# VinAIResearch/COMBAT

Hardware: AMD Instinct MI355X
Metric: images/sec per alternated generator+surrogate step, CIFAR-10 bs=128, 1/2/4/8 GPU (higher is better)
Workload: dtype bf16; 1 GPU; train_generator.py --dataset cifar10 --pc 0.5 --noise_rate 0.08: alternated PreActResNet18 surrogate + UNet generator step (Phase C + Phase G, both Nesterov-SGD updates), bs=128 per GPU, on-device augmentation on; per_gpu_batch=128, global_batch=128, parallelism=dp1 (RCCL all-reduce of netC grads in Phase C, netG grads in Phase G), losses_finite=True, deterministic=True

## Files before the change

### combat_amd/build.py

```python
import importlib.util
import os
import subprocess
import sys
from concurrent.futures import ThreadPoolExecutor

HERE = os.path.dirname(os.path.abspath(__file__))
ROOT = os.path.dirname(HERE)
CSRC = os.path.join(HERE, "csrc")
OBJ = os.path.join(CSRC, "_obj")
LIB = os.path.join(HERE, "libcombat_hip.so")
SOURCES = ["capi.cpp", "plan.cpp", "comm.cpp", "conv_gemm.hip", "conv3x3.hip", "conv3x3_dma.hip", "conv_gather_dma.hip", "conv_k8.hip", "conv_wgrad.hip", "conv_wgrad3x3.hip", "conv_wgrad3x3_dma.hip", "norm.hip", "elementwise.hip", "trigger.hip", "head.hip", "warp.hip"]
HIPCC = os.environ.get("HIPCC", "/opt/rocm/bin/hipcc")
FLAGS = ["--offload-arch=gfx950", "-O3", "-std=c++17", "-fPIC", "-munsafe-fp-atomics", "-Wno-unused-result", "-Wno-inline-asm",
         "-I" + os.path.join(ROOT, "include"), "-I" + CSRC] + os.environ.get("COMBAT_HIPCC_FLAGS", "").split()


def _newer(target, deps):
    if not os.path.exists(target):
        return True
    t = os.path.getmtime(target)
    return any(os.path.getmtime(d) > t for d in deps)


def check_counted_waits(lib=LIB, verbose=True):
    spec = importlib.util.spec_from_file_location("check_counted_waits", os.path.join(ROOT, "tools", "check_counted_waits.py"))
    mod = importlib.util.module_from_spec(spec)
    spec.loader.exec_module(mod)
    res = mod.check_file(lib)
    if verbose or not res.ok():
        print(res.report(), flush=True)
    if not res.ok():
        raise RuntimeError("counted-wait check failed: %d error(s), first: %s at 0x%x: %s"
                           % (len(res.errors), res.errors[0].kernel, res.errors[0].addr, res.errors[0].text))
    return res


def build(force=False, verbose=True):
    os.makedirs(OBJ, exist_ok=True)
    headers = [os.path.join(ROOT, "include", "combat_hip.h"), os.path.join(CSRC, "common.hpp"), os.path.join(CSRC, "conv_common.hpp"), os.path.join(CSRC, "conv_dma_epilogue.hpp"), os.path.join(CSRC, "plan.hpp")]
    jobs = []
    objs = []
    for src in SOURCES:
        s = os.path.join(CSRC, src)
        o = os.path.join(OBJ, os.path.splitext(src)[0] + ".o")
        objs.append(o)
        if force or _newer(o, [s] + headers):
            cmd = [HIPCC] + FLAGS + (["-x", "hip"] if src.endswith(".cpp") else []) + ["-c", s, "-o", o]
            jobs.append(cmd)

    def run(cmd):
        if verbose:
            print(" ".join(cmd), flush=True)
        subprocess.run(cmd, check=True)

    if jobs:
        with ThreadPoolExecutor(max_workers=min(4, len(jobs))) as ex:
            list(ex.map(run, jobs))
    if jobs or force or _newer(LIB, objs):
        tmp = LIB + ".unchecked"
        if os.path.exists(LIB):
            os.remove(LIB)
        run([HIPCC, "--offload-arch=gfx950", "-shared", "-fPIC", "-o", tmp] + objs)
        check_counted_waits(tmp, verbose)
        os.replace(tmp, LIB)
    return LIB


if __name__ == "__main__":
    print(build(force="--force" in sys.argv))
```

### combat_amd/csrc/conv_common.hpp

```cpp
#pragma once
#include "common.hpp"
#include <type_traits>

int conv3x3_pick(const combat_conv_args *a);
int conv3x3_stats_layout(const combat_conv_args *a, int tile, int *rows, int *rows_per_image);
int conv3x3_launch(const combat_conv_args *a, int tile, hipStream_t st);
int conv3x3d_pick(const combat_conv_args *a);
int conv3x3d_stats_layout(const combat_conv_args *a, int tile, int *rows, int *rows_per_image);
int conv3x3d_launch(const combat_conv_args *a, int tile, hipStream_t st);
int conv_gather_dma_bn(const combat_conv_args *a);
bool conv_gather_dma_parity_split(const combat_conv_args *a);
bool conv_c8_ok(const combat_conv_args *a);
int conv_c8_launch(const combat_conv_args *a, hipStream_t st);
bool conv_k8_ok(const combat_conv_args *a);
int conv_k8_launch(const combat_conv_args *a, hipStream_t st);
int conv_gather_dma_launch(const combat_conv_args *a, hipStream_t st);
int conv_gather_dma_pair_launch(const combat_conv_args *a, const combat_conv_args *b, hipStream_t st);
long conv_gather_dma_workspace(const combat_conv_args *a);
int conv_wgrad3x3_try(const combat_wgrad_args *a, hipStream_t st);
int conv_wgrad3x3_dma_try(const combat_wgrad_args *a, hipStream_t st);
long conv_wgrad3x3_dma_workspace(const combat_wgrad_args *a);
int conv_wgrad3x3_dma_reduce(const combat_wgrad_args *a, hipStream_t st);

template <int BM, int BN, int WGM_ = 0>
struct TileCfg {
    static constexpr int WGM = WGM_ ? WGM_ : ((BN == 16) ? 4 : 2);
    static constexpr int WGN = 4 / WGM;
    static constexpr int WM = BM / WGM;
    static constexpr int WN = BN / WGN;
    static constexpr int FM = WM / 16;
    static constexpr int FN = WN / 16;
    static constexpr int A_ITERS = BM / 32;
    static constexpr int B_ITERS = (BN + 31) / 32;
    static constexpr int EPS = BN + 4;
    static constexpr int STAGE_BYTES = 2 * (BM + BN) * 128;
    static constexpr int EP_BYTES = BM * EPS * 4;
    static constexpr int SMEM = STAGE_BYTES > EP_BYTES ? STAGE_BYTES : EP_BYTES;
    static constexpr int NC = BN / 8;
    static constexpr int RPT = BM * NC / 256;
    static constexpr int SG = BM / 4;
};

template <typename T, typename RowMap>
__device__ __forceinline__ void conv_epilogue(unsigned char *smem, const f32x4_t (&acc)[T::FN][T::FM],
                                              const combat_conv_args &a, int n0, int PQ, RowMap row_to_m,
                                              int part_row) {
    const int tid = threadIdx.x, lane = tid & 63, wid = tid >> 6;
    const int wave_m = wid % T::WGM, wave_n = wid / T::WGM;
    float *ep = reinterpret_cast<float *>(smem);
    {
        const int fr = lane & 15, fq = lane >> 4;
#pragma unroll
        for (int i = 0; i < T::FN; ++i)
#pragma unroll
            for (int j = 0; j < T::FM; ++j) {
                const int n = wave_n * T::WN + i * 16 + fq * 4;
                const int row = wave_m * T::WM + j * 16 + fr;
                *reinterpret_cast<f32x4_t *>(ep + row * T::EPS + n) = acc[i][j];
            }
    }
    __syncthreads();

    const int K = a.K;
    const int cc = tid % T::NC, rgrp = tid / T::NC;
    const int n = n0 + cc * 8;
    const bool n_ok = n < K;
    float bias8[8];
    if (a.bias && n_ok) load8f(a.bias + n, bias8);
    float s1[8], s2[8];
#pragma unroll
    for (int e = 0; e < 8; ++e) s1[e] = s2[e] = 0.f;
    __bf16 *__restrict__ dst = reinterpret_cast<__bf16 *>(a.dst);
    __bf16 *__restrict__ act_dst = reinterpret_cast<__bf16 *>(a.act_dst);
    float asc[8], ash[8];
    if (act_dst && n_ok) {
        load8f(a.act_scale + n, asc);
        load8f(a.act_shift + n, ash);
    }

    auto tail = [&](auto shared_tag) {
    constexpr bool tab_shared = decltype(shared_tag)::value;
    float msc[8], msh[8], hrs[8], hmn[8];
    if (a.mask_x && n_ok && tab_shared) {
        if (a.mask_scale) {
            load8f(a.mask_scale + n, msc);
            load8f(a.mask_shift + n, msh);
        }
        if ((a.stats_kind & 3) == 2) {
            load8f(a.xh_rstd + n, hrs);
            load8f(a.xh_mean + n, hmn);
        }
    }
    constexpr int RB = T::RPT < 4 ? T::RPT : 4;
#pragma unroll
    for (int pb = 0; pb < T::RPT; pb += RB) {
        int mrow[RB];
        uint4 l_pre[RB], l_x[RB], l_post[RB];
#pragma unroll
        for (int q = 0; q < RB; ++q) {
            const int row = rgrp * T::RPT + pb + q;
            const int m = n_ok ? row_to_m(row) : -1;
            mrow[q] = m;
            if (m >= 0) {
                const size_t off = (size_t)m * K + n;
                if (a.add_pre) l_pre[q] = *reinterpret_cast<const uint4 *>(reinterpret_cast<const __bf16 *>(a.add_pre) + off);
                if (a.mask_x) l_x[q] = *reinterpret_cast<const uint4 *>(reinterpret_cast<const __bf16 *>(a.mask_x) + off);
                if (a.add_post) l_post[q] = *reinterpret_cast<const uint4 *>(reinterpret_cast<const __bf16 *>(a.add_post) + off);
            }
        }
#pragma unroll
        for (int q = 0; q < RB; ++q) {
            const int m = mrow[q];
            if (m < 0) continue;
            const int row = rgrp * T::RPT + pb + q;
            float v[8];
            load8f(ep + row * T::EPS + cc * 8, v);
            const size_t off = (size_t)m * K + n;
            if (a.bias) {
#pragma unroll
                for (int e = 0; e < 8; ++e) v[e] += bias8[e];
            }
            if (a.add_pre) {
                float t[8];
                unpack8(l_pre[q], t);
#pragma unroll
                for (int e = 0; e < 8; ++e) v[e] += t[e];
            }
            float xm[8];
            if (a.mask_x) {
                unpack8(l_x[q], xm);
                if constexpr (!tab_shared) {
                    const int g = (m / PQ) * a.mask_group_stride;
                    if (a.mask_scale) {
                        load8f(a.mask_scale + g + n, msc);
                        load8f(a.mask_shift + g + n, msh);
                    }
                    if ((a.stats_kind & 3) == 2) {
                        load8f(a.xh_rstd + g + n, hrs);
                        load8f(a.xh_mean + g + n, hmn);
                    }
                }
                if (a.mask_scale) {
#pragma unroll
                    for (int e = 0; e < 8; ++e) {
                        const float qv = a.mask_activated ? xm[e] : fmaf(xm[e], msc[e], msh[e]);
                        float d = qv > 0.f ? 1.f : a.mask_slope;
                        if (a.mask_mul_scale) d *= msc[e];
                        v[e] *= d;
                    }
                } else {
#pragma unroll
                    for (int e = 0; e < 8; ++e) v[e] *= xm[e] > 0.f ? 1.f : a.mask_slope;
                }
            }
            if (a.add_post) {
                float t[8];
                unpack8(l_post[q], t);
#pragma unroll
                for (int e = 0; e < 8; ++e) v[e] += t[e];
            }
            if (a.tanh_out) {
#pragma unroll
                for (int e = 0; e < 8; ++e) v[e] = tanhf(v[e]);
            }
            const uint4 packed = pack8(v);
            if (dst) *reinterpret_cast<uint4 *>(dst + off) = packed;
            if (act_dst) {
                float t[8];
                unpack8(packed, t);
#pragma unroll
                for (int e = 0; e < 8; ++e) {
                    const float q = fmaf(t[e], asc[e], ash[e]);
                    t[e] = q > 0.f ? q : q * a.act_slope;
                }
                *reinterpret_cast<uint4 *>(act_dst + off) = pack8(t);
// ... 43 lines not shown
```

### combat_amd/csrc/conv_wgrad.hip

```cpp
#include "conv_common.hpp"
#include "plan.hpp"

namespace {

struct WgradParams {
    combat_wgrad_args a;
    int M, PQ, ntaps, tiles_k, tiles_c, split, pix_per_split;
    float *ws;
};

template <int BMC, int BNC>
struct WCfg {
    static constexpr int WGK = (BNC == 16) ? 4 : (BMC == 16 ? 1 : 2);
    static constexpr int WGC = 4 / WGK;
    static constexpr int WK = BMC / WGK;
    static constexpr int WC = BNC / WGC;
    static constexpr int FK = WK / 16;
    static constexpr int FC = WC / 16;
    static constexpr int SK = (BMC + 16) * 2;
    static constexpr int SC = (BNC + 16) * 2;
    static constexpr int CHK = BMC / 8;
    static constexpr int CHC = BNC / 8;
    static constexpr int ITK = (64 * CHK + 255) / 256;
    static constexpr int ITC = (64 * CHC + 255) / 256;
// ... 389 lines not shown
    p.ws = (p.split > 1 && p.a.workspace && p.a.workspace_bytes >= need) ? reinterpret_cast<float *>(p.a.workspace) : nullptr;
    if (combat_deterministic() && p.split > 1 && !p.ws) return COMBAT_EINVAL;
    COMBAT_LAUNCH(conv_wgrad_c8_kernel, dim3((unsigned)(p.tiles_k * p.split)), dim3(256), SMEM, st, p);
    CB_LAUNCH_CHECK();
    if (p.ws) {
        const int groups = p.split >= 32 ? 16 : 1;
        float *part = nullptr;
        if (combat_deterministic() && groups > 1) {
            const long extra = (long)groups * p.tiles_k * per_tile * 4;
            if (p.a.workspace_bytes >= need + extra) part = p.ws + need / 4;
        }
        const int g1 = combat_deterministic() && !part ? 1 : groups;
        COMBAT_LAUNCH(conv_wgrad_c8_reduce_kernel, dim3((per_tile + 255) / 256, p.tiles_k, g1), dim3(256), 0, st, (const float *)p.ws,
                           p.a.dw, p.tiles_k, p.split, per_tile, p.a.k_real, 9 * p.a.c_real, part);
        CB_LAUNCH_CHECK();
        if (part) {
            COMBAT_LAUNCH(conv_wgrad_c8_reduce_kernel, dim3((per_tile + 255) / 256, p.tiles_k, 1), dim3(256), 0, st, (const float *)part,
                               p.a.dw, p.tiles_k, groups, per_tile, p.a.k_real, 9 * p.a.c_real, (float *)nullptr);
            CB_LAUNCH_CHECK();
        }
    }
    return COMBAT_OK;
}

__global__ __launch_bounds__(256) void wgrad_slab_reduce_kernel(const float *__restrict__ ws, float *__restrict__ dw, int split,
                                                                int ntaps, int tiles_k, int tiles_c, int bmc, int bnc, int k_real,
                                                                int c_real, int C) {
    const long e = (long)blockIdx.x * 256 + threadIdx.x;
    if (e >= (long)k_real * ntaps * c_real) return;
    const int c = (int)(e % c_real), tap = (int)((e / c_real) % ntaps), n = (int)(e / ((long)c_real * ntaps));
    const int tile_k = n / bmc, row = n - tile_k * bmc;
    const size_t tile_elems = (size_t)bmc * bnc, sstride = (size_t)ntaps * tiles_k * tiles_c * tile_elems;
    float total = 0.f;
    for (int half = 0; half < 2; ++half) {
        const int cs = c + half * c_real;
        if (half && (c_real >= C || cs >= C || cs >= 2 * c_real)) break;
        const int tile_c = cs / bnc, col = cs - tile_c * bnc;
        const float *src = ws + (((size_t)tap * tiles_k + tile_k) * tiles_c + tile_c) * tile_elems + (size_t)row * bnc + col;
        float s0 = 0.f, s1 = 0.f, s2 = 0.f, s3 = 0.f;
        int sp = 0;
        for (; sp + 4 <= split; sp += 4) {
            s0 += src[(size_t)sp * sstride];
            s1 += src[(size_t)(sp + 1) * sstride];
            s2 += src[(size_t)(sp + 2) * sstride];
            s3 += src[(size_t)(sp + 3) * sstride];
        }
        for (; sp < split; ++sp) s0 += src[(size_t)sp * sstride];
        total += (s0 + s1) + (s2 + s3);
    }
    dw[e] += total;
}

template <int BMC, int BNC>
int64_t generic_slab_bytes(const combat_wgrad_args &a, int split) {
    const long tiles_k = (a.K + BMC - 1) / BMC, tiles_c = (a.C + BNC - 1) / BNC;
    return (int64_t)split * a.R * a.S * tiles_k * tiles_c * BMC * BNC * 4;
}

template <int BMC, int BNC>
int launch(WgradParams p, hipStream_t st) {
    using T = WCfg<BMC, BNC>;
    static bool attr_set = false;
    auto kern = conv_wgrad_kernel<BMC, BNC>;
    if (!attr_set) {
        if (hipFuncSetAttribute(reinterpret_cast<const void *>(kern), hipFuncAttributeMaxDynamicSharedMemorySize,
                                T::SMEM) != hipSuccess)
            return COMBAT_ELAUNCH;
        attr_set = true;
    }
    p.tiles_k = (p.a.K + BMC - 1) / BMC;
    p.tiles_c = (p.a.C + BNC - 1) / BNC;
    int split = p.a.split;
    const int ktiles = (p.M + 63) / 64;
    if (split <= 0) {
        const int base = p.tiles_k * p.tiles_c * p.ntaps;
        split = ((BMC == 16 ? 2304 : 256) + base - 1) / base;
        const int max_split = (ktiles + 3) / 4;
        if (split > max_split) split = max_split;
        if (split < 1) split = 1;
    }
    if (split > ktiles) split = ktiles;
    p.pix_per_split = ((ktiles + split - 1) / split) * 64;
    p.split = (p.M + p.pix_per_split - 1) / p.pix_per_split;
    const long blocks = (long)p.tiles_k * p.tiles_c * p.ntaps * p.split;
    p.ws = nullptr;
    if (combat_deterministic() && p.split > 1) {
        const int64_t need = generic_slab_bytes<BMC, BNC>(p.a, p.split);
        if (!p.a.workspace || p.a.workspace_bytes < need) return COMBAT_EINVAL;
        p.ws = reinterpret_cast<float *>(p.a.workspace);
    }
    COMBAT_LAUNCH(kern, dim3((unsigned)blocks), dim3(256), T::SMEM, st, p);
    CB_LAUNCH_CHECK();
    if (p.ws) {
        const long elems = (long)p.a.k_real * p.ntaps * p.a.c_real;
        COMBAT_LAUNCH(wgrad_slab_reduce_kernel, dim3((unsigned)((elems + 255) / 256)), dim3(256), 0, st, (const float *)p.ws, p.a.dw,
                      p.split, p.ntaps, p.tiles_k, p.tiles_c, BMC, BNC, p.a.k_real, p.a.c_real, p.a.C);
        CB_LAUNCH_CHECK();
    }
    return COMBAT_OK;
}

template <int BMC, int BNC>
int generic_split(const combat_wgrad_args &a) {
    const long M = (long)a.N * a.P * a.Q;
    const int ktiles = (int)((M + 63) / 64), ntaps = a.R * a.S;
    const int tiles_k = (a.K + BMC - 1) / BMC, tiles_c = (a.C + BNC - 1) / BNC;
    int split = a.split > 0 ? a.split : 0;
    if (split <= 0) {
        const int base = tiles_k * tiles_c * ntaps;
        split = ((BMC == 16 ? 2304 : 256) + base - 1) / base;
        const int max_split = (ktiles + 3) / 4;
        if (split > max_split) split = max_split;
        if (split < 1) split = 1;
    }
    if (split > ktiles) split = ktiles;
    const int pix_per_split = ((ktiles + split - 1) / split) * 64;
    return (int)((M + pix_per_split - 1) / pix_per_split);
}

bool c8_applies(const combat_wgrad_args *a) {
    return a->split >= 0 && a->C == 8 && a->R == 3 && (a->K & 63) == 0 && !a->pro_scale && !a->pro_act;
}

int64_t c8_workspace(const combat_wgrad_args &a) {
    const long M = (long)a.N * a.P * a.Q;
    const int ktiles = (int)((M + 63) / 64), tiles_k = a.K / 64;
    int split = a.split;
    if (split <= 0) {
        split = (256 + tiles_k - 1) / tiles_k;
        const int max_split = (ktiles + 3) / 4;
        if (split > max_split) split = max_split;
        if (split < 1) split = 1;
    }
    if (split > ktiles) split = ktiles;
    const int pix_per_split = ((ktiles + split - 1) / split) * 64;
    const long nsplit = (M + pix_per_split - 1) / pix_per_split;
    if (nsplit <= 1) return 0;
    const int64_t per_tile = 64 * 9 * a.c_real * 4;
    return tiles_k * nsplit * per_tile + (nsplit >= 32 ? 16 * tiles_k * per_tile : 0);
}

int64_t generic_workspace(const combat_wgrad_args &a) {
    if (a.C <= 16) return generic_slab_bytes<64, 16>(a, generic_split<64, 16>(a));
    if (a.K <= 16) return generic_slab_bytes<16, 64>(a, generic_split<16, 64>(a));
    if (a.C % 128 == 0 && a.K % 128 == 0) return generic_slab_bytes<128, 128>(a, generic_split<128, 128>(a));
    return generic_slab_bytes<64, 64>(a, generic_split<64, 64>(a));
}

}

extern "C" int64_t combat_conv_wgrad_workspace_bytes(const combat_wgrad_args *a) {
    if (!a) return 0;
    const int64_t dma = a->split >= 0 ? (int64_t)conv_wgrad3x3_dma_workspace(a) : 0;
    if (dma > 0 || !combat_deterministic()) return dma;
    return c8_applies(a) ? c8_workspace(*a) : generic_workspace(*a);
}

static int validate_wgrad_args(const combat_wgrad_args *a) {
    if (!a || !a->src || !a->dy || !a->dw) return COMBAT_EINVAL;
    if (a->N <= 0 || a->H <= 0 || a->W <= 0 || a->P <= 0 || a->Q <= 0) return COMBAT_EINVAL;
    if (a->C < 8 || (a->C & 7) || a->K < 8 || (a->K & 7)) return COMBAT_EINVAL;
    if (a->R != a->S || (a->R != 1 && a->R != 3)) return COMBAT_EINVAL;
    if (a->stride != 1 && a->stride != 2) return COMBAT_EINVAL;
    if (a->c_real <= 0 || a->c_real > a->C || a->k_real <= 0 || a->k_real > a->K) return COMBAT_EINVAL;
    if ((a->pro_scale == nullptr) != (a->pro_shift == nullptr)) return COMBAT_EINVAL;
    if ((long)a->N * a->P * a->Q > 0x7fffffffL / 8) return COMBAT_EINVAL;
    return COMBAT_OK;
}

extern "C" int combat_conv_wgrad_reduce(const combat_wgrad_args *a, void *stream) {
    COMBAT_PLAN_HOOK(combat_conv_wgrad_reduce, a);
    if (validate_wgrad_args(a) != COMBAT_OK) return COMBAT_EINVAL;
    if (a->split < 0 || !a->defer_reduce) return COMBAT_OK;
    return conv_wgrad3x3_dma_reduce(a, as_stream(stream));
}

extern "C" int combat_conv_wgrad(const combat_wgrad_args *a, void *stream) {
    COMBAT_PLAN_HOOK(combat_conv_wgrad, a);
    if (validate_wgrad_args(a) != COMBAT_OK) return COMBAT_EINVAL;
    WgradParams p;
    p.a = *a;
    p.ws = nullptr;
    p.PQ = a->P * a->Q;
    p.M = (int)((long)a->N * p.PQ);
    p.ntaps = a->R * a->S;
    hipStream_t st = as_stream(stream);
    if (a->split >= 0) {
        int rc = conv_wgrad3x3_dma_try(a, st);
        if (rc <= 0) return rc;
    }
    if (a->reduce_first) {
        const int rc = combat_conv_wgrad_reduce(a->reduce_first, stream);
        if (rc != COMBAT_OK) return rc;
    }
    if (a->split >= 0 && !combat_deterministic()) {
        const int rc = conv_wgrad3x3_try(a, st);
        if (rc <= 0) return rc;
    }
    if (a->split < 0) p.a.split = 0;
    if (c8_applies(a)) return launch_c8(p, st);
    if (a->C <= 16) return launch<64, 16>(p, st);
    if (a->K <= 16) return launch<16, 64>(p, st);
    if (a->C % 128 == 0 && a->K % 128 == 0) return launch<128, 128>(p, st);
    return launch<64, 64>(p, st);
}
```

### combat_amd/csrc/conv_wgrad3x3_dma.hip

```cpp
#include "conv_common.hpp"
#include <stdlib.h>

namespace {

typedef __attribute__((address_space(3))) void lds_void_t;
constexpr unsigned kOob = 0x40000000u;

struct W3dParams {
    combat_wgrad_args a;
    int TW, TH, TI, HWP, HH, HROWS, hpw, tw_shift, th_shift;
    int tiles_x, tiles_y, ntiles, tiles_k, tiles_c, split, per;
    unsigned x_bytes, dy_bytes;
    float *ws;
    const float *red_ws;
    float *red_dw;
    int red_base, red_tiles_c, red_split, red_k_real, red_c_real, red_pad;
    unsigned long long *stamps;
};

#ifdef COMBAT_STAMPS
static unsigned long long *g_stamps_wgrad_host = nullptr;
extern "C" int combat_debug_set_stamps_wgrad(void *p) { g_stamps_wgrad_host = (unsigned long long *)p; return 0; }
#define WCLK() __builtin_readcyclecounter()
#else
// ... 423 lines not shown
__global__ __launch_bounds__(512, 1) void conv_wgrad3x3_dma_kernel(const W3dParams p) { wgrad3x3_dma_body<HPW, NS, RED>(p); }

template <int HPW, int NS, bool RED>
int launch_w3d_red(const W3dParams &p, int blocks, hipStream_t st) {
    constexpr int stage = 8192 + HPW * 8192;
    constexpr int ep = 64 * 68 * 4;
    constexpr int smem = NS * stage > ep ? NS * stage : ep;
    auto kern = conv_wgrad3x3_dma_kernel<HPW, NS, RED>;
    static bool attr = false;
    if (!attr) {
        if (hipFuncSetAttribute(reinterpret_cast<const void *>(kern), hipFuncAttributeMaxDynamicSharedMemorySize, smem) != hipSuccess)
            return COMBAT_ELAUNCH;
        attr = true;
    }
    COMBAT_LAUNCH(kern, dim3(blocks), dim3(512), smem, st, p);
    CB_LAUNCH_CHECK();
    return COMBAT_OK;
}

template <int HPW, int NS>
int launch_w3d(const W3dParams &p, int blocks, hipStream_t st) {
    return p.red_ws ? launch_w3d_red<HPW, NS, true>(p, blocks, st) : launch_w3d_red<HPW, NS, false>(p, blocks, st);
}

bool w3d_geometry(const combat_wgrad_args *a, W3dParams &p, int &smem) {
    if (!(a->R == 3 && a->S == 3 && a->stride == 1 && a->pad == 1 && a->P == a->H && a->Q == a->W)) return false;
    if (a->pro_scale || a->pro_act) return false;
    if (a->C < 64 || (a->C & 63) || a->K < 64 || (a->K & 63) || a->c_real != a->C) return false;
    const int W = a->W, H = a->H;
    const int TW = W < 16 ? W : 16;
    const int TH = H < 64 / TW ? H : 64 / TW;
    const int TI = 64 / (TW * TH);
    if (TW < 2 || TI < 1 || TW * TH * TI != 64) return false;
    p.a = *a;
    p.TW = TW; p.TH = TH; p.TI = TI;
    p.HWP = TW + 2; p.HH = TH + 2; p.HROWS = TI * p.HH * p.HWP;
    p.hpw = (p.HROWS + 63) / 64;
    p.tw_shift = ilog2_exact(TW); p.th_shift = ilog2_exact(TH);
    if (p.tw_shift < 0 || p.th_shift < 0 || W % TW || H % TH) return false;
    const long xb = (long)a->N * H * W * a->C * 2, db = (long)a->N * H * W * a->K * 2;
    if (xb >= (long)kOob || db >= (long)kOob) return false;
    p.x_bytes = (unsigned)xb; p.dy_bytes = (unsigned)db;
    p.tiles_x = W / TW; p.tiles_y = H / TH;
    p.ntiles = p.tiles_x * p.tiles_y * ((a->N + TI - 1) / TI);
    p.tiles_k = a->K / 64; p.tiles_c = a->C / 64;
    smem = 0;
    return p.hpw >= 2 && p.hpw <= 4;
}

int pick_split(const combat_wgrad_args *a, const W3dParams &p, bool with_ws) {
    const int base = p.tiles_k * p.tiles_c;
    int split = a->split;
    if (split <= 0) {
        static const int ws_wgs = getenv("COMBAT_WGRAD_WGS") ? atoi(getenv("COMBAT_WGRAD_WGS")) : 128;
        const int by_cus = ((with_ws ? ws_wgs : 256) + base - 1) / base;
        const int by_atomics = 164 / base > 0 ? 164 / base : 1;
        split = with_ws || by_cus < by_atomics ? by_cus : by_atomics;
        const int by_work = (p.ntiles + 3) / 4;
        if (split > by_work) split = by_work;
        if (split < 1) split = 1;
    }
    if (split > p.ntiles) split = p.ntiles;
    const int per = (p.ntiles + split - 1) / split;
    return (p.ntiles + per - 1) / per;
}

}

long conv_wgrad3x3_dma_workspace(const combat_wgrad_args *a) {
    W3dParams p;
    int smem;
    if (!w3d_geometry(a, p, smem)) return 0;
    const int split = pick_split(a, p, true);
    return split > 1 ? (long)split * p.tiles_k * p.tiles_c * 9 * 4096 * 4 : 0;
}

namespace {
bool w3d_plan(const combat_wgrad_args *a, W3dParams &p) {
    int smem;
    if (!w3d_geometry(a, p, smem)) return false;
    const int base = p.tiles_k * p.tiles_c;
    int split = pick_split(a, p, true);
    const bool use_ws = split > 1 && a->workspace && a->workspace_bytes >= (long)split * base * 9 * 4096 * 4;
    if (!use_ws) split = pick_split(a, p, false);
    p.ws = use_ws ? reinterpret_cast<float *>(a->workspace) : nullptr;
    p.per = (p.ntiles + split - 1) / split;
    p.split = (p.ntiles + p.per - 1) / p.per;
    return true;
}

int launch_reduce(const combat_wgrad_args *a, const W3dParams &p, hipStream_t st) {
    const int base = p.tiles_k * p.tiles_c;
    static const bool env_det = getenv("COMBAT_WGRAD_DET_REDUCE") != nullptr;
    const bool det = combat_deterministic();
    const bool atomics = !env_det && (!det || base >= 4);
    if (atomics) {
        const long e4 = (long)base * 9 * 1024;
        int groups = (int)(512 / ((e4 + 255) / 256));
        if (groups < 1 || det) groups = 1;
        if (groups > p.split) groups = p.split;
        COMBAT_LAUNCH(wgrad3x3_reduce_kernel, dim3((unsigned)((e4 + 255) / 256), groups), dim3(256), 0, st, p.ws, a->dw, base,
                           p.tiles_c, p.split, a->k_real, a->c_real);
    } else {
        COMBAT_LAUNCH(wgrad3x3_reduce_det_kernel, dim3(256), dim3(256), 0, st, (const float *)p.ws, a->dw, base, p.tiles_c, p.split,
                           a->k_real, a->c_real);
    }
    CB_LAUNCH_CHECK();
    return COMBAT_OK;
}

bool fill_reduce_first(const combat_wgrad_args *prev, W3dParams &p) {
    p.red_ws = nullptr;
    p.red_dw = nullptr;
    p.red_base = p.red_tiles_c = p.red_split = p.red_k_real = p.red_c_real = p.red_pad = 0;
    if (!prev) return true;
    W3dParams q;
    if (!w3d_plan(prev, q)) return true;
    if (!q.ws) return true;
    p.red_ws = q.ws;
    p.red_dw = prev->dw;
    p.red_base = q.tiles_k * q.tiles_c;
    p.red_tiles_c = q.tiles_c;
    p.red_split = q.split;
    p.red_k_real = prev->k_real;
    p.red_c_real = prev->c_real;
    return true;
}
}

int conv_wgrad3x3_dma_try(const combat_wgrad_args *a, hipStream_t st) {
    W3dParams p;
    if (!w3d_plan(a, p)) return 1;
    if (combat_deterministic() && !p.ws && p.split > 1) return COMBAT_EINVAL;
    if (!fill_reduce_first(a->reduce_first, p)) return COMBAT_EINVAL;
#ifdef COMBAT_STAMPS
    p.stamps = g_stamps_wgrad_host;
#else
    p.stamps = nullptr;
#endif
    const int blocks = p.tiles_k * p.tiles_c * p.split;
    int rc;
    if (p.hpw == 2) rc = launch_w3d<2, 3>(p, blocks, st);
    else if (p.hpw == 3) rc = launch_w3d<3, 2>(p, blocks, st);
    else rc = launch_w3d<4, 2>(p, blocks, st);
    if (rc != COMBAT_OK || !p.ws || a->defer_reduce) return rc;
    return launch_reduce(a, p, st);
}

int conv_wgrad3x3_dma_reduce(const combat_wgrad_args *a, hipStream_t st) {
    W3dParams p;
    if (!w3d_plan(a, p) || !p.ws) return COMBAT_OK;
    return launch_reduce(a, p, st);
}
```

Baseline: 32970 images/sec.

## Add DMA-fed MFMA weight-gradient kernel for stride-2 3x3 convolutions

Adds a dedicated weight-gradient kernel for stride-2, pad-1 3x3 convolutions. It uses buffer-load-to-LDS DMA with a two-stage ring, parity-split input columns, swizzled LDS layouts and transposed LDS reads feeding bf16 MFMA. Partial results go to per-split workspace slabs that are reduced deterministically by the existing slab-reduce kernel. This replaces the generic or c8 GEMM path for the PreActResNet and UNet downsampling convs, at the cost of more workspace and a separate reduce launch.

```diff
diff --git a/combat_amd/build.py b/combat_amd/build.py
--- a/combat_amd/build.py
+++ b/combat_amd/build.py
@@ -9,7 +9,7 @@
 CSRC = os.path.join(HERE, "csrc")
 OBJ = os.path.join(CSRC, "_obj")
 LIB = os.path.join(HERE, "libcombat_hip.so")
-SOURCES = ["capi.cpp", "plan.cpp", "comm.cpp", "conv_gemm.hip", "conv3x3.hip", "conv3x3_dma.hip", "conv_gather_dma.hip", "conv_k8.hip", "conv_wgrad.hip", "conv_wgrad3x3.hip", "conv_wgrad3x3_dma.hip", "norm.hip", "elementwise.hip", "trigger.hip", "head.hip", "warp.hip"]
+SOURCES = ["capi.cpp", "plan.cpp", "comm.cpp", "conv_gemm.hip", "conv3x3.hip", "conv3x3_dma.hip", "conv_gather_dma.hip", "conv_k8.hip", "conv_wgrad.hip", "conv_wgrad3x3.hip", "conv_wgrad3x3_dma.hip", "conv_wgrad3x3_s2_dma.hip", "norm.hip", "elementwise.hip", "trigger.hip", "head.hip", "warp.hip"]
 HIPCC = os.environ.get("HIPCC", "/opt/rocm/bin/hipcc")
 FLAGS = ["--offload-arch=gfx950", "-O3", "-std=c++17", "-fPIC", "-munsafe-fp-atomics", "-Wno-unused-result", "-Wno-inline-asm",
          "-I" + os.path.join(ROOT, "include"), "-I" + CSRC] + os.environ.get("COMBAT_HIPCC_FLAGS", "").split()
diff --git a/combat_amd/csrc/conv_common.hpp b/combat_amd/csrc/conv_common.hpp
--- a/combat_amd/csrc/conv_common.hpp
+++ b/combat_amd/csrc/conv_common.hpp
@@ -21,6 +21,9 @@
 int conv_wgrad3x3_dma_try(const combat_wgrad_args *a, hipStream_t st);
 long conv_wgrad3x3_dma_workspace(const combat_wgrad_args *a);
 int conv_wgrad3x3_dma_reduce(const combat_wgrad_args *a, hipStream_t st);
+int conv_wgrad3x3_slab_reduce(const combat_wgrad_args *a, float *ws, int tiles_k, int tiles_c, int split, hipStream_t st);
+int conv_wgrad3x3_s2_dma_try(const combat_wgrad_args *a, hipStream_t st);
+long conv_wgrad3x3_s2_dma_workspace(const combat_wgrad_args *a);
 
 template <int BM, int BN, int WGM_ = 0>
 struct TileCfg {
diff --git a/combat_amd/csrc/conv_wgrad.hip b/combat_amd/csrc/conv_wgrad.hip
--- a/combat_amd/csrc/conv_wgrad.hip
+++ b/combat_amd/csrc/conv_wgrad.hip
@@ -565,7 +565,10 @@
 extern "C" int64_t combat_conv_wgrad_workspace_bytes(const combat_wgrad_args *a) {
     if (!a) return 0;
     const int64_t dma = a->split >= 0 ? (int64_t)conv_wgrad3x3_dma_workspace(a) : 0;
-    if (dma > 0 || !combat_deterministic()) return dma;
+    if (dma > 0) return dma;
+    const int64_t s2 = a->split >= 0 ? (int64_t)conv_wgrad3x3_s2_dma_workspace(a) : -1;
+    if (s2 >= 0) return s2;
+    if (!combat_deterministic()) return dma;
     return c8_applies(a) ? c8_workspace(*a) : generic_workspace(*a);
 }
 
@@ -606,6 +609,10 @@
         const int rc = combat_conv_wgrad_reduce(a->reduce_first, stream);
         if (rc != COMBAT_OK) return rc;
     }
+    if (a->split >= 0) {
+        const int rc = conv_wgrad3x3_s2_dma_try(a, st);
+        if (rc <= 0) return rc;
+    }
     if (a->split >= 0 && !combat_deterministic()) {
         const int rc = conv_wgrad3x3_try(a, st);
         if (rc <= 0) return rc;
diff --git a/combat_amd/csrc/conv_wgrad3x3_dma.hip b/combat_amd/csrc/conv_wgrad3x3_dma.hip
--- a/combat_amd/csrc/conv_wgrad3x3_dma.hip
+++ b/combat_amd/csrc/conv_wgrad3x3_dma.hip
@@ -599,3 +599,12 @@
     if (!w3d_plan(a, p) || !p.ws) return COMBAT_OK;
     return launch_reduce(a, p, st);
 }
+
+int conv_wgrad3x3_slab_reduce(const combat_wgrad_args *a, float *ws, int tiles_k, int tiles_c, int split, hipStream_t st) {
+    W3dParams p{};
+    p.ws = ws;
+    p.tiles_k = tiles_k;
+    p.tiles_c = tiles_c;
+    p.split = split;
+    return launch_reduce(a, p, st);
+}
diff --git a/combat_amd/csrc/conv_wgrad3x3_s2_dma.hip b/combat_amd/csrc/conv_wgrad3x3_s2_dma.hip
--- /dev/null
+++ b/combat_amd/csrc/conv_wgrad3x3_s2_dma.hip
@@ -0,0 +1,376 @@
+#include "conv_common.hpp"
+#include <stdlib.h>
+
+namespace {
+
+typedef __attribute__((address_space(3))) void lds_void_t;
+typedef __attribute__((address_space(3))) unsigned char lds_u8;
+constexpr unsigned kOob = 0x40000000u;
+
+struct W3sParams {
+    combat_wgrad_args a;
+    int TW, TH, TI, HWP, HH, HROWS, hpw, tw_shift, th_shift;
+    int tiles_x, tiles_y, ntiles, tiles_k, tiles_c, split, per;
+    unsigned x_bytes, dy_bytes;
+    float *ws;
+};
+
+__device__ __forceinline__ s16x4_t tr16s(const lds_u8 *p) {
+    return __builtin_amdgcn_ds_read_tr16_b64_v4i16((__attribute__((address_space(3))) s16x4_t *)(const_cast<lds_u8 *>(p)));
+}
+
+__device__ __forceinline__ bf16x8_t join8s(const s16x4_t lo, const s16x4_t hi) {
+    typedef __attribute__((ext_vector_type(8))) short s16x8_t;
+    const s16x8_t v = {lo[0], lo[1], lo[2], lo[3], hi[0], hi[1], hi[2], hi[3]};
+    return __builtin_bit_cast(bf16x8_t, v);
+}
+
+__device__ __forceinline__ int xslot(int TW, int hx) { return (hx & 1) ? TW + 1 + (hx >> 1) : (hx >> 1); }
+__device__ __forceinline__ int xkey(int TW, int line, int cx) {
+    return ((cx >> 1) & 1) | ((TW == 16 ? (cx >> 3) & 1 : TW == 8 ? (line >> 1) & 1 : (line >> 2) & 1) << 1);
+}
+__device__ __forceinline__ int dkey(int pk) { return ((pk >> 1) & 1) | (((pk >> 3) & 1) << 1); }
+
+__device__ __forceinline__ void drain_barrier() {
+    asm volatile("s_waitcnt vmcnt(0) lgkmcnt(0)" ::: "memory");
+    __builtin_amdgcn_s_barrier();
+    asm volatile("" ::: "memory");
+}
+
+template <int HPW>
+__device__ __forceinline__ void wgrad3x3_s2_body(const W3sParams &p) {
+    extern __shared__ __attribute__((aligned(16))) unsigned char smem[];
+    constexpr int NS = 2;
+    const combat_wgrad_args &a = p.a;
+    const int tid = threadIdx.x, lane = tid & 63;
+    const int wid = __builtin_amdgcn_readfirstlane(tid >> 6);
+    const int wave_k = wid & 1, wave_c = wid >> 1;
+    int bid = blockIdx.x;
+    const int tile_c = bid % p.tiles_c; bid /= p.tiles_c;
+    const int tile_k = bid % p.tiles_k;
+    const int sp = bid / p.tiles_k;
+    const int k0 = tile_k * 64, c0 = tile_c * 64;
+    const int t_begin = sp * p.per;
+    int t_end = t_begin + p.per;
+    if (t_end > p.ntiles) t_end = p.ntiles;
+    if (t_begin >= t_end) return;
+
+    const int C = a.C, K = a.K, H = a.H, W = a.W, P = a.P, Q = a.Q;
+    constexpr int XBYTES = HPW * 8 * 1024, DYBYTES = 64 * 128, DYBASE = NS * XBYTES;
+    static_assert((NS - 1) * XBYTES < 65536, "slot offset as a ds_read immediate");
+    auto rsrc_words = [&](const void *ptr, unsigned bytes) __attribute__((always_inline)) {
+        const unsigned long base = (unsigned long)ptr;
+        u32x4_t w;
+        w[0] = __builtin_amdgcn_readfirstlane((unsigned)base);
+        w[1] = __builtin_amdgcn_readfirstlane((unsigned)(base >> 32) & 0xffffu);
+        w[2] = __builtin_amdgcn_readfirstlane(bytes);
+        w[3] = 0x00020000u;
+        return w;
+    };
+    const u32x4_t xrs = rsrc_words(a.src, p.x_bytes), dyrs = rsrc_words(a.dy, p.dy_bytes);
+    const unsigned lds0 = __builtin_amdgcn_readfirstlane((unsigned)(unsigned long)(lds_void_t *)smem) + wid * 1024;
+#define COMBAT_W3S_DMA(rs_words, lds_off, voff) \
+    asm volatile("s_mov_b32 m0, %0\n\ts_nop 0\n\tbuffer_load_dwordx4 %1, %2, 0 offen lds" ::"s"(lds0_l + (unsigned)(lds_off)), "v"(voff), "s"(rs_words##_l) : "memory", "m0")
+
+    int hdec[HPW], hrel[HPW];
+#pragma unroll
+    for (int j = 0; j < HPW; ++j) {
+        const int row = (wid + 8 * j) * 8 + (lane >> 3), slot = lane & 7;
+        const int cx = row % p.HWP, lrow = row / p.HWP;
+        const int line = lrow % p.HH, ti = lrow / p.HH;
+        const int hx = cx <= p.TW ? 2 * cx : 2 * (cx - p.TW - 1) + 1;
+        const int chunk = (((slot >> 1) ^ xkey(p.TW, line, cx)) << 1) | (slot & 1);
+        hdec[j] = row < p.HROWS ? (hx | (line << 8) | (ti << 16)) : -1;
+        hrel[j] = (((ti * H + line - 1) * W + hx - 1) * C + c0 + chunk * 8) * 2;
+        asm volatile("" : "+v"(hdec[j]), "+v"(hrel[j]));
+    }
+    int dti, drel;
+    {
+        const int pk = wid * 8 + (lane >> 3), slot = lane & 7;
+        const int tx = pk & (p.TW - 1), ty = (pk >> p.tw_shift) & (p.TH - 1), ti = pk >> (p.tw_shift + p.th_shift);
+        const int chunk = (((slot >> 1) ^ dkey(pk)) << 1) | (slot & 1);
+        dti = ti;
+        drel = (((ti * P + ty) * Q + tx) * K + k0 + chunk * 8) * 2;
+        asm volatile("" : "+v"(dti), "+v"(drel));
+    }
+    int nt_x, nt_y, nt_g;
+    {
+        const int t = t_begin;
+        nt_x = t % p.tiles_x;
+        nt_y = (t / p.tiles_x) % p.tiles_y;
+        nt_g = t / (p.tiles_x * p.tiles_y);
+    }
+    int is_img0 = 0, is_iy0 = 0, is_ix0 = 0, is_xorg = 0, is_dorg = 0;
+    auto issue_prep = [&]() __attribute__((always_inline)) {
+        is_img0 = nt_g * p.TI;
+        const int oy0 = nt_y * p.TH, ox0 = nt_x * p.TW;
+        is_iy0 = 2 * oy0;
+        is_ix0 = 2 * ox0;
+        is_xorg = ((is_img0 * H + is_iy0) * W + is_ix0) * C * 2;
+        is_dorg = ((is_img0 * P + oy0) * Q + ox0) * K * 2;
+        if (++nt_x == p.tiles_x) {
+            nt_x = 0;
+            if (++nt_y == p.tiles_y) {
+                nt_y = 0;
+                ++nt_g;
+            }
+        }
+    };
+    auto issue_piece = [&](auto j_tag, auto slot_tag) __attribute__((always_inline)) {
+        constexpr int j = decltype(j_tag)::value;
+        constexpr int slot_i = decltype(slot_tag)::value;
+        const u32x4_t xrs_l = xrs, dyrs_l = dyrs;
+        const unsigned lds0_l = lds0;
+        (void)xrs_l; (void)dyrs_l; (void)lds0_l;
+        if constexpr (j == 0) {
+            const unsigned off = is_img0 + dti < a.N ? (unsigned)(is_dorg + drel) : kOob;
+            COMBAT_W3S_DMA(dyrs, DYBASE + slot_i * DYBYTES, off);
+        } else if constexpr (j <= HPW) {
+            const int d = hdec[j - 1];
+            const bool ok = d >= 0 && is_img0 + (d >> 16) < a.N && (unsigned)(is_iy0 + ((d >> 8) & 255) - 1) < (unsigned)H &&
+                            (unsigned)(is_ix0 + (d & 255) - 1) < (unsigned)W;
+            const unsigned off = ok ? (unsigned)(is_xorg + hrel[j - 1]) : kOob;
+            COMBAT_W3S_DMA(xrs, slot_i * XBYTES + 8 * (j - 1) * 1024, off);
+        }
+    };
+    auto issue = [&](auto slot_tag) __attribute__((always_inline)) {
+        using std::integral_constant;
+        issue_prep();
+        issue_piece(integral_constant<int, 0>{}, slot_tag);
+        issue_piece(integral_constant<int, 1>{}, slot_tag);
+        issue_piece(integral_constant<int, 2>{}, slot_tag);
+        issue_piece(integral_constant<int, 3>{}, slot_tag);
+        issue_piece(integral_constant<int, 4>{}, slot_tag);
+        issue_piece(integral_constant<int, 5>{}, slot_tag);
+        issue_piece(integral_constant<int, 6>{}, slot_tag);
+    };
+    static_assert(HPW <= 6, "issue() spells out 1 + HPW <= 7 pieces");
+
+    const int q = (lane & 15) >> 2, pp = lane & 3, fq = lane >> 4;
+    const lds_u8 *const smem_l = (const lds_u8 *)smem;
+    const lds_u8 *dyp[2][2][2], *xp[2][2][9];
+#pragma unroll
+    for (int ks = 0; ks < 2; ++ks)
+#pragma unroll
+        for (int hi = 0; hi < 2; ++hi) {
+            const int pk = ks * 32 + fq * 8 + q + 4 * hi;
+            const int dya = pk * 128 + ((wave_k ^ dkey(pk)) & 3) * 32 + pp * 8;
+            const int tx = pk & (p.TW - 1), ty = (pk >> p.tw_shift) & (p.TH - 1), ti = pk >> (p.tw_shift + p.th_shift);
+#pragma unroll
+            for (int tap = 0; tap < 9; ++tap) {
+                const int r = (tap * 11) >> 5, s = tap - 3 * r;
+                const int line = 2 * ty + r, cx = xslot(p.TW, 2 * tx + s);
+                const int xa = ((ti * p.HH + line) * p.HWP + cx) * 128 + ((wave_c ^ xkey(p.TW, line, cx)) & 3) * 32 + pp * 8;
+                xp[ks][hi][tap] = smem_l + xa;
+                asm volatile("" : "+v"(xp[ks][hi][tap]));
+            }
+#pragma unroll
+            for (int i = 0; i < 2; ++i) {
+                dyp[ks][hi][i] = smem_l + DYBASE + (dya ^ (i * 64));
+                asm volatile("" : "+v"(dyp[ks][hi][i]));
+            }
+        }
+
+    f32x4_t acc[9][2];
+#pragma unroll
+    for (int t = 0; t < 9; ++t)
+#pragma unroll
+        for (int i = 0; i < 2; ++i) acc[t][i] = f32x4_t{0.f, 0.f, 0.f, 0.f};
+
+    auto x_frags = [&](bf16x8_t (&fx)[2], auto slot_tag, auto tap_tag) __attribute__((always_inline)) {
+        constexpr int tap = decltype(tap_tag)::value, imm = decltype(slot_tag)::value * XBYTES;
+#pragma unroll
+        for (int ks = 0; ks < 2; ++ks) fx[ks] = join8s(tr16s(xp[ks][0][tap] + imm), tr16s(xp[ks][1][tap] + imm));
+    };
+    auto mfma_tap = [&](auto tap_tag, const bf16x8_t (&fk)[2][2], const bf16x8_t (&fx)[2]) __attribute__((always_inline)) {
+        constexpr int tap = decltype(tap_tag)::value;
+#pragma unroll
+        for (int ks = 0; ks < 2; ++ks)
+#pragma unroll
+            for (int i = 0; i < 2; ++i)
+                acc[tap][i] = __builtin_amdgcn_mfma_f32_16x16x32_bf16(fk[ks][i], fx[ks], acc[tap][i], 0, 0, 0);
+        if (tap < 8) {
+#pragma unroll
+            for (int r = 0; r < 4; ++r) {
+                __builtin_amdgcn_sched_group_barrier(0x008, 1, 0);
+                __builtin_amdgcn_sched_group_barrier(0x100, 1, 0);
+            }
+        }
+        __builtin_amdgcn_sched_barrier(0);
+    };
+    auto compute = [&](auto slot_tag) __attribute__((always_inline)) {
+        constexpr int imm = decltype(slot_tag)::value * DYBYTES;
+        bf16x8_t fk[2][2];
+#pragma unroll
+        for (int ks = 0; ks < 2; ++ks)
+#pragma unroll
+            for (int i = 0; i < 2; ++i)
+                fk[ks][i] = join8s(tr16s(dyp[ks][0][i] + imm), tr16s(dyp[ks][1][i] + imm));
+        using std::integral_constant;
+        bf16x8_t fx0[2], fx1[2];
+        x_frags(fx0, slot_tag, integral_constant<int, 0>{});
+        __builtin_amdgcn_sched_barrier(0);
+#define COMBAT_W3S_TAP(t, cur, nxt)                                                  \
+        if (t < 8) x_frags(nxt, slot_tag, integral_constant<int, (t < 8 ? t + 1 : 8)>{});  \
+        mfma_tap(integral_constant<int, t>{}, fk, cur);
+        COMBAT_W3S_TAP(0, fx0, fx1) COMBAT_W3S_TAP(1, fx1, fx0) COMBAT_W3S_TAP(2, fx0, fx1) COMBAT_W3S_TAP(3, fx1, fx0)
+        COMBAT_W3S_TAP(4, fx0, fx1) COMBAT_W3S_TAP(5, fx1, fx0) COMBAT_W3S_TAP(6, fx0, fx1) COMBAT_W3S_TAP(7, fx1, fx0)
+        COMBAT_W3S_TAP(8, fx0, fx1)
+#undef COMBAT_W3S_TAP
+    };
+
+    const int npatch = t_end - t_begin;
+    using std::integral_constant;
+    issue(integral_constant<int, 0>{});
+    drain_barrier();
+    auto body = [&](auto slot_tag, int i) __attribute__((always_inline)) {
+        constexpr int slot = decltype(slot_tag)::value;
+        if (i + 1 < npatch) issue(integral_constant<int, slot ^ 1>{});
+        __builtin_amdgcn_sched_barrier(0);
+        compute(slot_tag);
+        drain_barrier();
+    };
+    for (int i = 0; i < npatch; i += 2) {
+        body(integral_constant<int, 0>{}, i);
+        if (i + 1 < npatch) body(integral_constant<int, 1>{}, i + 1);
+    }
+#undef COMBAT_W3S_DMA
+
+    if (p.ws) {
+        float *slab = p.ws + (size_t)blockIdx.x * 9 * 4096;
+#pragma unroll
+        for (int tap = 0; tap < 9; ++tap)
+#pragma unroll
+            for (int i = 0; i < 2; ++i)
+                *reinterpret_cast<f32x4_t *>(slab + tap * 4096 + ((i * 8 + wid) * 64 + lane) * 4) = acc[tap][i];
+    } else {
+        float *ep = reinterpret_cast<float *>(smem);
+        constexpr int EPS = 68;
+        const int fr = lane & 15;
+#pragma unroll 1
+        for (int tap = 0; tap < 9; ++tap) {
+#pragma unroll
+            for (int i = 0; i < 2; ++i) {
+                const int col = wave_c * 16 + fr;
+                const int row = (i * 2 + wave_k) * 16 + fq * 4;
+                f32x4_t v;
+                switch (tap) {
+                    case 0: v = acc[0][i]; break;
+                    case 1: v = acc[1][i]; break;
+                    case 2: v = acc[2][i]; break;
+                    case 3: v = acc[3][i]; break;
+                    case 4: v = acc[4][i]; break;
+                    case 5: v = acc[5][i]; break;
+                    case 6: v = acc[6][i]; break;
+                    case 7: v = acc[7][i]; break;
+                    default: v = acc[8][i]; break;
+                }
+#pragma unroll
+                for (int e = 0; e < 4; ++e) ep[(row + e) * EPS + col] = v[e];
+            }
+            __syncthreads();
+            for (int idx = tid; idx < 64 * 64; idx += 512) {
+                const int row = idx >> 6, col = idx & 63;
+                const int n = k0 + row, c = c0 + col;
+                if (n < a.k_real && c < a.c_real) atomicAdd(a.dw + ((size_t)n * 9 + tap) * a.c_real + c, ep[row * EPS + col]);
+            }
+            __syncthreads();
+        }
+    }
+}
+
+template <int HPW, int NS>
+__global__ __launch_bounds__(512, 1) void conv_wgrad3x3_dma_s2_kernel(const W3sParams p) {
+    static_assert(NS == 2, "a ring of two stages: every wait is a drain");
+    wgrad3x3_s2_body<HPW>(p);
+}
+
+template <int HPW>
+int launch_w3s(const W3sParams &p, int blocks, hipStream_t st) {
+    constexpr int smem = 2 * (8192 + HPW * 8192);
+    auto kern = conv_wgrad3x3_dma_s2_kernel<HPW, 2>;
+    static bool attr = false;
+    if (!attr) {
+        if (hipFuncSetAttribute(reinterpret_cast<const void *>(kern), hipFuncAttributeMaxDynamicSharedMemorySize, smem) != hipSuccess)
+            return COMBAT_ELAUNCH;
+        attr = true;
+    }
+    COMBAT_LAUNCH(kern, dim3(blocks), dim3(512), smem, st, p);
+    CB_LAUNCH_CHECK();
+    return COMBAT_OK;
+}
+
+bool w3s_geometry(const combat_wgrad_args *a, W3sParams &p) {
+    if (!(a->R == 3 && a->S == 3 && a->stride == 2 && a->pad == 1)) return false;
+    if ((a->H & 1) || (a->W & 1) || a->P * 2 != a->H || a->Q * 2 != a->W) return false;
+    if (a->pro_scale || a->pro_act) return false;
+    if (a->C < 64 || (a->C & 63) || a->K < 64 || (a->K & 63) || a->c_real != a->C) return false;
+    const int P = a->P, Q = a->Q;
+    const int TW = Q < 16 ? Q : 16;
+    const int TH = P < 64 / TW ? P : 64 / TW;
+    if (TW < 4 || TH < 1) return false;
+    const int TI = 64 / (TW * TH);
+    if (TI < 1 || TW * TH * TI != 64) return false;
+    p.a = *a;
+    p.TW = TW; p.TH = TH; p.TI = TI;
+    p.HWP = 2 * TW + 1; p.HH = 2 * TH + 1; p.HROWS = TI * p.HH * p.HWP;
+    p.hpw = (p.HROWS + 63) / 64;
+    p.tw_shift = ilog2_exact(TW); p.th_shift = ilog2_exact(TH);
+    if (p.tw_shift < 0 || p.th_shift < 0 || Q % TW || P % TH) return false;
+    if (TW == 4 && TH != 4) return false;
+    const long xb = (long)a->N * a->H * a->W * a->C * 2, db = (long)a->N * P * Q * a->K * 2;
+    if (xb >= (long)kOob || db >= (long)kOob) return false;
+    p.x_bytes = (unsigned)xb; p.dy_bytes = (unsigned)db;
+    p.tiles_x = Q / TW; p.tiles_y = P / TH;
+    p.ntiles = p.tiles_x * p.tiles_y * ((a->N + TI - 1) / TI);
+    p.tiles_k = a->K / 64; p.tiles_c = a->C / 64;
+    return p.hpw >= 1 && p.hpw <= 6;
+}
+
+int pick_split(const combat_wgrad_args *a, const W3sParams &p, bool with_ws) {
+    const int base = p.tiles_k * p.tiles_c;
+    int split = a->split;
+    if (split <= 0) {
+        static const int ws_wgs = getenv("COMBAT_WGRAD_WGS") ? atoi(getenv("COMBAT_WGRAD_WGS")) : 128;
+        const int by_cus = ((with_ws ? ws_wgs : 256) + base - 1) / base;
+        const int by_atomics = 164 / base > 0 ? 164 / base : 1;
+        split = with_ws || by_cus < by_atomics ? by_cus : by_atomics;
+        const int by_work = (p.ntiles + 3) / 4;
+        if (split > by_work) split = by_work;
+        if (split < 1) split = 1;
+    }
+    if (split > p.ntiles) split = p.ntiles;
+    const int per = (p.ntiles + split - 1) / split;
+    return (p.ntiles + per - 1) / per;
+}
+
+bool w3s_plan(const combat_wgrad_args *a, W3sParams &p) {
+    if (!w3s_geometry(a, p)) return false;
+    const int base = p.tiles_k * p.tiles_c;
+    int split = pick_split(a, p, true);
+    const bool use_ws = split > 1 && a->workspace && a->workspace_bytes >= (long)split * base * 9 * 4096 * 4;
+    if (!use_ws) split = pick_split(a, p, false);
+    p.ws = use_ws ? reinterpret_cast<float *>(a->workspace) : nullptr;
+    p.per = (p.ntiles + split - 1) / split;
+    p.split = (p.ntiles + p.per - 1) / p.per;
+    return true;
+}
+
+}
+
+long conv_wgrad3x3_s2_dma_workspace(const combat_wgrad_args *a) {
+    W3sParams p;
+    if (!w3s_geometry(a, p)) return -1;
+    const int split = pick_split(a, p, true);
+    return split > 1 ? (long)split * p.tiles_k * p.tiles_c * 9 * 4096 * 4 : 0;
+}
+
+int conv_wgrad3x3_s2_dma_try(const combat_wgrad_args *a, hipStream_t st) {
+    W3sParams p;
+    if (!w3s_plan(a, p)) return 1;
+    if (combat_deterministic() && !p.ws && p.split > 1) return COMBAT_EINVAL;
+    const int blocks = p.tiles_k * p.tiles_c * p.split;
+    const int rc = p.hpw <= 5 ? launch_w3s<5>(p, blocks, st) : launch_w3s<6>(p, blocks, st);
+    if (rc != COMBAT_OK || !p.ws) return rc;
+    return conv_wgrad3x3_slab_reduce(a, p.ws, p.tiles_k, p.tiles_c, p.split, st);
+}
```

Result: no change. 33070 images/sec (median of 2 runs) (+0.3%).
